# mayuelala/FollowYourClick

Measured on AMD Instinct MI355X. Metric: denoised frames/sec, 16f x 512^2 clip @ 25 DDIM steps, higher is better.
Workload: dtype bf16; 1 GPU; configs[1]: AnimationPipeline DDIM loop, SD-1.5 UNet3D + mm_sd_v15-shaped motion modules (random init), 1 clip/GPU of 16 frames 512x512, 25 DDIM steps, CFG 8.0, mask + first-frame concat, fps/flow conditioning; frames=16, height=512, width=512, ddim_steps=25, parallelism=dp1 (independent clips, weight broadcast 0.00 GiB in 0.00s)

## Files before the change

### followyourclick_amd/csrc/panel_linear.hip

```cpp
#include <mutex>

#include "chan_parts.h"
#include "fyc_common.h"

namespace {

constexpr int ROWS = 128, NT = 256, PN = 320;
constexpr int NB = PN / 16;
constexpr int PIECE = 1024;
constexpr int NPIECE = 2 * NB;
constexpr int STAGE_BYTES = NPIECE * PIECE;
constexpr int RING_BYTES = 2 * STAGE_BYTES;
constexpr int TILE_BYTES = ROWS * PN * 2;
constexpr int LDS_BYTES = RING_BYTES + TILE_BYTES;
static_assert(LDS_BYTES <= 160 * 1024, "LDS budget");

struct PLP {
  const bf16_t* x; const bf16_t* res; bf16_t* out;
  const char* ws;
  const float* bias;
  const double* gn_cs;
  ChanParts gn_parts;
  const float* gn_gamma; const float* gn_beta;
  int gn_rows_per_sample, gn_stat_samples, gn_groups;
  float gn_eps;
  int N;
};

__device__ __forceinline__ void dma16(const char* gbase, unsigned voff, unsigned lds_dst) {
  unsigned keep;
  asm volatile("s_mov_b32 %0, m0\n\ts_mov_b32 m0, %3\n\ts_nop 0\n\tglobal_load_lds_dwordx4 %1, %2\n\ts_mov_b32 m0, %0"
               : "=&s"(keep) : "v"(voff), "s"(gbase), "s"(lds_dst) : "memory");
}
__device__ __forceinline__ void dma16v(const void* gsrc, unsigned lds_dst) {
  unsigned keep;
  asm volatile("s_mov_b32 %0, m0\n\ts_mov_b32 m0, %2\n\ts_nop 0\n\tglobal_load_lds_dwordx4 %1, off\n\ts_mov_b32 m0, %0"
               : "=&s"(keep) : "v"(gsrc), "s"(lds_dst) : "memory");
}
__device__ __forceinline__ void dma_landed_barrier() {
  asm volatile("s_waitcnt vmcnt(0)" ::: "memory");
  __syncthreads();
}
__device__ __forceinline__ f32x4 mfma(bf16x8 a, bf16x8 b, f32x4 c) { return __builtin_amdgcn_mfma_f32_16x16x32_bf16(a, b, c, 0, 0, 0); }
__device__ __forceinline__ f32x4 mfma(f16x8 a, f16x8 b, f32x4 c) { return __builtin_amdgcn_mfma_f32_16x16x32_f16(a, b, c, 0, 0, 0); }
template <typename Frag> __device__ __forceinline__ Frag frag(const char* sl, int piece) { return *reinterpret_cast<const Frag*>(sl + piece * PIECE); }

template <typename E16, int KS, int NPASS>
__global__ void __launch_bounds__(NT) panel_linear_kernel(const PLP p) {
  typedef typename Pair16<E16>::Vec8 Frag;
  constexpr int K = KS * 32, SPP = KS / 2;
  extern __shared__ __attribute__((aligned(16))) char smem[];
  char* const tile = smem + RING_BYTES;
  const int tid = threadIdx.x, lane = tid & 63;
  const int wave = __builtin_amdgcn_readfirstlane(tid >> 6);
  const int g = lane >> 4, r16 = lane & 15;
  const unsigned lane16 = (unsigned)lane * 16u;
  const unsigned lds0 = (unsigned)(size_t)(__attribute__((address_space(3))) char*)smem;
  const long long row0 = (long long)blockIdx.x * ROWS;

  auto dma_piece = [&](int T, int n) {
    const int q = wave + 4 * n;
    dma16(p.ws + (long long)T * STAGE_BYTES + q * PIECE, lane16, lds0 + (T & 1) * STAGE_BYTES + q * PIECE);
  };

  Frag xa[2][KS];
  {
    const bf16_t* xr = p.x + (row0 + wave * 32 + r16) * K + g * 8;
#pragma unroll
    for (int i = 0; i < 2; ++i)
#pragma unroll
      for (int s = 0; s < KS; ++s) xa[i][s] = *reinterpret_cast<const Frag*>(xr + (long long)i * 16 * K + s * 32);
  }
#pragma unroll
  for (int n = 0; n < 10; ++n) dma_piece(0, n);

  if (p.gn_cs != nullptr || p.gn_parts.parts != nullptr) {
    double* dsum = reinterpret_cast<double*>(tile);
    float* tab = reinterpret_cast<float*>(tile + K * 16);
    const int sample = (int)(row0 / p.gn_rows_per_sample), cpg = K / p.gn_groups;
    ChanPartsRange pr = {};
    if (p.gn_parts.parts != nullptr) pr = chan_parts_range(p.gn_parts, sample, p.gn_stat_samples);
    for (int c = tid; c < K; c += NT) {
      double s = 0.0, q = 0.0;
      if (p.gn_parts.parts != nullptr) {
        fold_chan_parts(p.gn_parts, pr, K, c, s, q);
      } else {
        for (int f = 0; f < p.gn_stat_samples; ++f) {
          const double* src = p.gn_cs + (((long long)sample * p.gn_stat_samples + f) * K + c) * 2;
          s += src[0]; q += src[1];
        }
      }
      dsum[2 * c] = s; dsum[2 * c + 1] = q;
    }
    __syncthreads();
    for (int c = tid; c < K; c += NT) {
      const int c0 = (c / cpg) * cpg;
      double s = 0.0, q = 0.0;
      for (int j = 0; j < cpg; ++j) { s += dsum[2 * (c0 + j)]; q += dsum[2 * (c0 + j) + 1]; }
      const double inv_cnt = 1.0 / ((double)p.gn_rows_per_sample * cpg);
      const double mean = s * inv_cnt;
      double var = q * inv_cnt - mean * mean;
      var = var > 0.0 ? var : 0.0;
      const float rstd = (float)(1.0 / sqrt(var + (double)p.gn_eps));
      const float sc = rstd * p.gn_gamma[c];
      tab[2 * c] = sc;
      tab[2 * c + 1] = p.gn_beta[c] - (float)mean * sc;
    }
    __syncthreads();
#pragma unroll
    for (int s = 0; s < KS; ++s) {
      float sc[8], sh[8];
#pragma unroll
      for (int e = 0; e < 8; e += 2) {
        const f32x4 t = *reinterpret_cast<const f32x4*>(tab + 2 * (32 * s + 8 * g + e));
        sc[e] = t[0]; sh[e] = t[1]; sc[e + 1] = t[2]; sh[e + 1] = t[3];
      }
#pragma unroll
      for (int i = 0; i < 2; ++i) {
        u32x4 t = __builtin_bit_cast(u32x4, xa[i][s]);
#pragma unroll
        for (int e = 0; e < 4; ++e)
          t[e] = Pair16<E16>::pack(__builtin_fmaf(Pair16<E16>::lo(t[e]), sc[2 * e], sh[2 * e]),
                                 __builtin_fmaf(Pair16<E16>::hi(t[e]), sc[2 * e + 1], sh[2 * e + 1]));
        xa[i][s] = __builtin_bit_cast(Frag, t);
      }
    }
    __syncthreads();
  }

  f32x4 oacc[2][NB];
#pragma unroll
  for (int pass = 0; pass < NPASS; ++pass) {
#pragma unroll
    for (int i = 0; i < 2; ++i)
#pragma unroll
      for (int j = 0; j < NB; ++j) oacc[i][j] = (f32x4){0.f, 0.f, 0.f, 0.f};
#pragma unroll
    for (int st = 0; st < SPP; ++st) {
      const int T = pass * SPP + st;
      dma_landed_barrier();
      if (st == SPP - 1 && p.res != nullptr) {
#pragma unroll
        for (int n = 0; n < TILE_BYTES / PIECE / 4; ++n) {
          const int c = (wave + 4 * n) * 64 + lane, row = c / 40, cg = c - row * 40;
          dma16v(p.res + (row0 + row) * p.N + pass * PN + cg * 8, lds0 + RING_BYTES + (wave + 4 * n) * PIECE);
        }
      }
      const char* sl = smem + (T & 1) * STAGE_BYTES + lane16;
#pragma unroll
      for (int u = 0; u < 2 * NB; ++u) {
        const int sk = u / NB, j = u % NB;
        const Frag wf = frag<Frag>(sl, u);
#pragma unroll
        for (int i = 0; i < 2; ++i) oacc[i][j] = mfma(wf, xa[i][2 * st + sk], oacc[i][j]);
        if (u < 10 && T + 1 < NPASS * SPP) dma_piece(T + 1, u);
      }
    }
    dma_landed_barrier();
#pragma unroll
    for (int i = 0; i < 2; ++i)
#pragma unroll
      for (int j = 0; j < NB; ++j) {
        E16* a = reinterpret_cast<E16*>(tile + (wave * 32 + i * 16 + r16) * (PN * 2)) + j * 16 + g * 4;
        f32x4 bo = {0.f, 0.f, 0.f, 0.f};
        if (p.bias != nullptr) bo = *reinterpret_cast<const f32x4*>(p.bias + pass * PN + j * 16 + g * 4);
        float rr[4] = {0.f, 0.f, 0.f, 0.f}, v[4];
        if (p.res != nullptr) ElemIO<E16>::ld4(a, rr);
#pragma unroll
        for (int r = 0; r < 4; ++r) v[r] = oacc[i][j][r] + bo[r] + rr[r];
        ElemIO<E16>::st4(a, v);
      }
    __syncthreads();
    {
      const int cg = tid % 40, rsl = tid / 40;
      if (rsl < 6) {
        char* dst = reinterpret_cast<char*>(p.out + row0 * p.N + pass * PN) + cg * 16;
        const char* src = tile + cg * 16;
#pragma unroll 2
        for (int row = rsl; row < ROWS; row += 6)
          *reinterpret_cast<u32x4*>(dst + (long long)row * p.N * 2) = *reinterpret_cast<const u32x4*>(src + row * (PN * 2));
      }
    }
    if (pass + 1 < NPASS) __syncthreads();
  }
}

template <typename T, int KS, int NPASS>
int launch(const PLP& p, int rows, hipStream_t st) {
  auto kern = panel_linear_kernel<T, KS, NPASS>;
  {
    constexpr int kMaxDev = 64;
    static std::mutex mu;
    static bool attr_done[kMaxDev] = {};
    int dev = 0;
    (void)hipGetDevice(&dev);
    std::lock_guard<std::mutex> lk(mu);
    if (dev < 0 || dev >= kMaxDev || !attr_done[dev]) {
      const hipError_t e = hipFuncSetAttribute(reinterpret_cast<const void*>(kern), hipFuncAttributeMaxDynamicSharedMemorySize, LDS_BYTES);
      if (e != hipSuccess) FYC_FAIL(-3, "fyc_panel_linear: %d bytes of dynamic LDS refused: %s", LDS_BYTES, hipGetErrorString(e));
      if (dev >= 0 && dev < kMaxDev) attr_done[dev] = true;
    }
  }
  hipLaunchKernelGGL(kern, dim3((unsigned)(rows / ROWS)), dim3(NT), LDS_BYTES, st, p);
  FYC_CHECK_LAUNCH("fyc_panel_linear");
  return 0;
}

}

extern "C" int64_t fyc_panel_linear_wstream_bytes(int32_t N, int32_t K) {
  if (N <= 0 || K <= 0 || N % PN != 0 || K % 64 != 0) return 0;
  return (int64_t)(N / PN) * (K / 64) * STAGE_BYTES;
}

extern "C" int fyc_panel_linear_supported(const fyc_panel_linear_args* a) {
  if (a == nullptr || (a->dtype != FYC_BF16 && a->dtype != FYC_F16) || a->rows <= 0 || a->rows % ROWS != 0) return 0;
  if (!((a->K == 320 || a->K == 640) && (a->N == 320 || a->N == 640))) return 0;
  if (a->gn_cs != nullptr && a->gn_parts != nullptr) return 0;
  if (a->gn_parts != nullptr && (a->gn_tile_rows <= 0 || a->gn_slots < 1 || a->gn_slots > 4 || a->gn_stat_samples <= 0 || a->gn_rows_per_sample % a->gn_stat_samples != 0)) return 0;
  if ((a->gn_cs != nullptr || a->gn_parts != nullptr) && (a->gn_rows_per_sample <= 0 || a->gn_rows_per_sample % ROWS != 0 || a->rows % a->gn_rows_per_sample != 0 ||
                              a->gn_groups <= 0 || a->K % a->gn_groups != 0 || a->gn_stat_samples <= 0)) return 0;
  static std::mutex mu;
  static int64_t lds_cap = -1;
  {
    std::lock_guard<std::mutex> lk(mu);
    if (lds_cap < 0) {
      int64_t caps[8];
      lds_cap = (fyc_device_caps(caps) == 0) ? caps[1] : 0;
    }
  }
  return (lds_cap > 0 && lds_cap < LDS_BYTES) ? 0 : 1;
}

extern "C" int fyc_panel_linear(const fyc_panel_linear_args* a, void* stream) {
  FYC_REQUIRE(a && a->x && a->out && a->wstream, "fyc_panel_linear: null pointer");
  FYC_REQUIRE(fyc_panel_linear_supported(a), "fyc_panel_linear: built for bf16 / f16, rows %% 128 == 0, K and N in {320, 640}, GroupNorm samples of whole 128-row tiles (got rows=%d K=%d N=%d gn_rows_per_sample=%d)",
              a->rows, a->K, a->N, a->gn_rows_per_sample);
  FYC_REQUIRE((a->gn_cs == nullptr && a->gn_parts == nullptr) || (a->gn_gamma != nullptr && a->gn_beta != nullptr), "fyc_panel_linear: gn_cs / gn_parts need gn_gamma / gn_beta");
  FYC_REQUIRE(a->x != a->out && a->residual != a->x, "fyc_panel_linear: out must not alias x (residual may alias out)");
  FYC_REQUIRE(((uintptr_t)a->x % 16) == 0 && ((uintptr_t)a->out % 16) == 0 && ((uintptr_t)a->wstream % 16) == 0 && ((uintptr_t)a->bias % 16) == 0 &&
              ((uintptr_t)a->residual % 16) == 0 && ((uintptr_t)a->gn_cs % 16) == 0 && ((uintptr_t)a->gn_parts % 8) == 0, "fyc_panel_linear: operands must be 16-byte aligned");
  PLP p;
  p.x = (const bf16_t*)a->x; p.res = (const bf16_t*)a->residual; p.out = (bf16_t*)a->out; p.ws = (const char*)a->wstream; p.bias = a->bias;
  p.gn_cs = a->gn_cs; p.gn_gamma = a->gn_gamma; p.gn_beta = a->gn_beta; p.gn_rows_per_sample = a->gn_rows_per_sample;
  p.gn_stat_samples = a->gn_stat_samples; p.gn_groups = a->gn_groups; p.gn_eps = a->gn_eps; p.N = a->N;
  p.gn_parts = ChanParts{a->gn_parts, a->gn_tile_rows, a->gn_slots, a->gn_parts != nullptr ? a->gn_rows_per_sample / a->gn_stat_samples : 1, a->rows};
  hipStream_t st = (hipStream_t)stream;
  if (a->dtype == FYC_F16) {
    if (a->K == 320) return a->N == 320 ? launch<f16_t, 10, 1>(p, a->rows, st) : launch<f16_t, 10, 2>(p, a->rows, st);
    return a->N == 320 ? launch<f16_t, 20, 1>(p, a->rows, st) : launch<f16_t, 20, 2>(p, a->rows, st);
  }
  if (a->K == 320) return a->N == 320 ? launch<bf16_t, 10, 1>(p, a->rows, st) : launch<bf16_t, 10, 2>(p, a->rows, st);
  return a->N == 320 ? launch<bf16_t, 20, 1>(p, a->rows, st) : launch<bf16_t, 20, 2>(p, a->rows, st);
}
```

Measured before the change: 14.40 frames/s.

## Halve panel-linear row tile to fit two workgroups per CU

Result: no change. 14.45 frames/s (median of 6 runs) (+0.4%).

```diff
diff --git a/followyourclick_amd/csrc/panel_linear.hip b/followyourclick_amd/csrc/panel_linear.hip
--- a/followyourclick_amd/csrc/panel_linear.hip
+++ b/followyourclick_amd/csrc/panel_linear.hip
@@ -5,15 +5,17 @@
 
 namespace {
 
-constexpr int ROWS = 128, NT = 256, PN = 320;
+constexpr int ROWS = 64, NT = 256, PN = 320;
+constexpr int ROW_ALIGN = 128;
 constexpr int NB = PN / 16;
 constexpr int PIECE = 1024;
-constexpr int NPIECE = 2 * NB;
+constexpr int NPIECE = NB;
 constexpr int STAGE_BYTES = NPIECE * PIECE;
 constexpr int RING_BYTES = 2 * STAGE_BYTES;
 constexpr int TILE_BYTES = ROWS * PN * 2;
 constexpr int LDS_BYTES = RING_BYTES + TILE_BYTES;
-static_assert(LDS_BYTES <= 160 * 1024, "LDS budget");
+static_assert(2 * LDS_BYTES <= 160 * 1024, "LDS budget: two workgroups per CU");
+static_assert(ROW_ALIGN % ROWS == 0, "a workgroup lies inside one GroupNorm sample");
 
 struct PLP {
   const bf16_t* x; const bf16_t* res; bf16_t* out;
@@ -46,9 +48,9 @@
 template <typename Frag> __device__ __forceinline__ Frag frag(const char* sl, int piece) { return *reinterpret_cast<const Frag*>(sl + piece * PIECE); }
 
 template <typename E16, int KS, int NPASS>
-__global__ void __launch_bounds__(NT) panel_linear_kernel(const PLP p) {
+__global__ void __launch_bounds__(NT, 2) panel_linear_kernel(const PLP p) {
   typedef typename Pair16<E16>::Vec8 Frag;
-  constexpr int K = KS * 32, SPP = KS / 2;
+  constexpr int K = KS * 32, SPP = KS;
   extern __shared__ __attribute__((aligned(16))) char smem[];
   char* const tile = smem + RING_BYTES;
   const int tid = threadIdx.x, lane = tid & 63;
@@ -63,16 +65,14 @@
     dma16(p.ws + (long long)T * STAGE_BYTES + q * PIECE, lane16, lds0 + (T & 1) * STAGE_BYTES + q * PIECE);
   };
 
-  Frag xa[2][KS];
+  Frag xa[1][KS];
   {
-    const bf16_t* xr = p.x + (row0 + wave * 32 + r16) * K + g * 8;
-#pragma unroll
-    for (int i = 0; i < 2; ++i)
-#pragma unroll
-      for (int s = 0; s < KS; ++s) xa[i][s] = *reinterpret_cast<const Frag*>(xr + (long long)i * 16 * K + s * 32);
-  }
-#pragma unroll
-  for (int n = 0; n < 10; ++n) dma_piece(0, n);
+    const bf16_t* xr = p.x + (row0 + wave * 16 + r16) * K + g * 8;
+#pragma unroll
+    for (int s = 0; s < KS; ++s) xa[0][s] = *reinterpret_cast<const Frag*>(xr + s * 32);
+  }
+#pragma unroll
+  for (int n = 0; n < NPIECE / 4; ++n) dma_piece(0, n);
 
   if (p.gn_cs != nullptr || p.gn_parts.parts != nullptr) {
     double* dsum = reinterpret_cast<double*>(tile);
@@ -115,26 +115,21 @@
         const f32x4 t = *reinterpret_cast<const f32x4*>(tab + 2 * (32 * s + 8 * g + e));
         sc[e] = t[0]; sh[e] = t[1]; sc[e + 1] = t[2]; sh[e + 1] = t[3];
       }
-#pragma unroll
-      for (int i = 0; i < 2; ++i) {
-        u32x4 t = __builtin_bit_cast(u32x4, xa[i][s]);
-#pragma unroll
-        for (int e = 0; e < 4; ++e)
-          t[e] = Pair16<E16>::pack(__builtin_fmaf(Pair16<E16>::lo(t[e]), sc[2 * e], sh[2 * e]),
-                                 __builtin_fmaf(Pair16<E16>::hi(t[e]), sc[2 * e + 1], sh[2 * e + 1]));
-        xa[i][s] = __builtin_bit_cast(Frag, t);
-      }
-    }
-    __syncthreads();
-  }
-
-  f32x4 oacc[2][NB];
+      u32x4 t = __builtin_bit_cast(u32x4, xa[0][s]);
+#pragma unroll
+      for (int e = 0; e < 4; ++e)
+        t[e] = Pair16<E16>::pack(__builtin_fmaf(Pair16<E16>::lo(t[e]), sc[2 * e], sh[2 * e]),
+                               __builtin_fmaf(Pair16<E16>::hi(t[e]), sc[2 * e + 1], sh[2 * e + 1]));
+      xa[0][s] = __builtin_bit_cast(Frag, t);
+    }
+    __syncthreads();
+  }
+
+  f32x4 oacc[1][NB];
 #pragma unroll
   for (int pass = 0; pass < NPASS; ++pass) {
 #pragma unroll
-    for (int i = 0; i < 2; ++i)
-#pragma unroll
-      for (int j = 0; j < NB; ++j) oacc[i][j] = (f32x4){0.f, 0.f, 0.f, 0.f};
+    for (int j = 0; j < NB; ++j) oacc[0][j] = (f32x4){0.f, 0.f, 0.f, 0.f};
 #pragma unroll
     for (int st = 0; st < SPP; ++st) {
       const int T = pass * SPP + st;
@@ -148,28 +143,23 @@
       }
       const char* sl = smem + (T & 1) * STAGE_BYTES + lane16;
 #pragma unroll
-      for (int u = 0; u < 2 * NB; ++u) {
-        const int sk = u / NB, j = u % NB;
-        const Frag wf = frag<Frag>(sl, u);
-#pragma unroll
-        for (int i = 0; i < 2; ++i) oacc[i][j] = mfma(wf, xa[i][2 * st + sk], oacc[i][j]);
-        if (u < 10 && T + 1 < NPASS * SPP) dma_piece(T + 1, u);
+      for (int j = 0; j < NB; ++j) {
+        oacc[0][j] = mfma(frag<Frag>(sl, j), xa[0][st], oacc[0][j]);
+        if (j < NPIECE / 4 && T + 1 < NPASS * SPP) dma_piece(T + 1, j);
       }
     }
     dma_landed_barrier();
 #pragma unroll
-    for (int i = 0; i < 2; ++i)
-#pragma unroll
-      for (int j = 0; j < NB; ++j) {
-        E16* a = reinterpret_cast<E16*>(tile + (wave * 32 + i * 16 + r16) * (PN * 2)) + j * 16 + g * 4;
-        f32x4 bo = {0.f, 0.f, 0.f, 0.f};
-        if (p.bias != nullptr) bo = *reinterpret_cast<const f32x4*>(p.bias + pass * PN + j * 16 + g * 4);
-        float rr[4] = {0.f, 0.f, 0.f, 0.f}, v[4];
-        if (p.res != nullptr) ElemIO<E16>::ld4(a, rr);
-#pragma unroll
-        for (int r = 0; r < 4; ++r) v[r] = oacc[i][j][r] + bo[r] + rr[r];
-        ElemIO<E16>::st4(a, v);
-      }
+    for (int j = 0; j < NB; ++j) {
+      E16* a = reinterpret_cast<E16*>(tile + (wave * 16 + r16) * (PN * 2)) + j * 16 + g * 4;
+      f32x4 bo = {0.f, 0.f, 0.f, 0.f};
+      if (p.bias != nullptr) bo = *reinterpret_cast<const f32x4*>(p.bias + pass * PN + j * 16 + g * 4);
+      float rr[4] = {0.f, 0.f, 0.f, 0.f}, v[4];
+      if (p.res != nullptr) ElemIO<E16>::ld4(a, rr);
+#pragma unroll
+      for (int r = 0; r < 4; ++r) v[r] = oacc[0][j][r] + bo[r] + rr[r];
+      ElemIO<E16>::st4(a, v);
+    }
     __syncthreads();
     {
       const int cg = tid % 40, rsl = tid / 40;
@@ -210,15 +200,15 @@
 
 extern "C" int64_t fyc_panel_linear_wstream_bytes(int32_t N, int32_t K) {
   if (N <= 0 || K <= 0 || N % PN != 0 || K % 64 != 0) return 0;
-  return (int64_t)(N / PN) * (K / 64) * STAGE_BYTES;
+  return (int64_t)(N / PN) * (K / 32) * STAGE_BYTES;
 }
 
 extern "C" int fyc_panel_linear_supported(const fyc_panel_linear_args* a) {
-  if (a == nullptr || (a->dtype != FYC_BF16 && a->dtype != FYC_F16) || a->rows <= 0 || a->rows % ROWS != 0) return 0;
+  if (a == nullptr || (a->dtype != FYC_BF16 && a->dtype != FYC_F16) || a->rows <= 0 || a->rows % ROW_ALIGN != 0) return 0;
   if (!((a->K == 320 || a->K == 640) && (a->N == 320 || a->N == 640))) return 0;
   if (a->gn_cs != nullptr && a->gn_parts != nullptr) return 0;
   if (a->gn_parts != nullptr && (a->gn_tile_rows <= 0 || a->gn_slots < 1 || a->gn_slots > 4 || a->gn_stat_samples <= 0 || a->gn_rows_per_sample % a->gn_stat_samples != 0)) return 0;
-  if ((a->gn_cs != nullptr || a->gn_parts != nullptr) && (a->gn_rows_per_sample <= 0 || a->gn_rows_per_sample % ROWS != 0 || a->rows % a->gn_rows_per_sample != 0 ||
+  if ((a->gn_cs != nullptr || a->gn_parts != nullptr) && (a->gn_rows_per_sample <= 0 || a->gn_rows_per_sample % ROW_ALIGN != 0 || a->rows % a->gn_rows_per_sample != 0 ||
                               a->gn_groups <= 0 || a->K % a->gn_groups != 0 || a->gn_stat_samples <= 0)) return 0;
   static std::mutex mu;
   static int64_t lds_cap = -1;
```
